# AMReX-Fluids/IAMR

Measured on AMD Instinct MI355X. Metric: cells-advanced/sec, higher is better.
Workload: dtype f64; 1 GPU; TaylorGreen 3D single level, one 256^3 box per GPU in a 1x1x1 arrangement (256x256x256 cells), periodic, nu=1e-4 cfl=0.7 Godunov_PLM be_cn_theta=0.5, full NavierStokes::advance per step

## Files before the change

iamr_amd/csrc/k_abec.hip:

```cpp
#include "kernels.h"
#include "launch.h"
#include <map>
#include <array>
#include <cstring>
#include <vector>
#include <algorithm>

namespace iamrx {

struct CfC1 { double c1[3][3]; double c2[3][3], c3[3][3]; int maxorder; int maintain; };

__device__ __forceinline__ void cf_maintain(const FabD& phi, const FabD& cfm, const BoxD& b, const CfC1& t, int i, int j, int k, double pnew)
{
    const int idx[3] = {i, j, k};
    for (int d = 0; d < 3; ++d) {
        const int NX = min(b.len(d) + 1, t.maxorder);
        if (NX < 2) continue;
        const int target = NX == 2 ? 1 : 2;
        for (int side = 0; side < 2; ++side) {
            const int s = side == 0 ? 1 : -1, f = side == 0 ? b.lo[d] : b.hi[d];
            if ((idx[d] - f) * s + 1 != target) continue;
            int g[3] = {i, j, k};
            g[d] = f - s;
            if (cfm(g[0], g[1], g[2]) != 1.0) continue;
// ... 496 lines not shown
}

__device__ __forceinline__ double rb_take(double v) { double r; asm volatile("v_mov_b64 %0, %1" : "=v"(r) : "v"(v)); return r; }

struct RbBC { int per[3]; double c1lo[3], c2lo[3], c1hi[3], c2hi[3]; int dlo[3], dhi[3]; double c3lo[3] = {0.0, 0.0, 0.0}, c3hi[3] = {0.0, 0.0, 0.0}; };
#ifndef IAMRX_RBW_EXP
#define IAMRX_RBW_EXP 0
#endif

template <bool SG, bool WALLS>
__device__ __forceinline__ double rb_update(double dhx, double dhy, double dhz, double omega,
    double p0, double pxm, double pxp, double pym, double pyp, double pzm, double pzp, double rr, double aa,
    double bxm, double bxp, double bym, double byp, double bzm, double bzp,
    double cxl, double cxh, double cyl, double cyh, double czl, double czh)
{
    const double gamma = aa + dhx * (bxm + bxp) + dhy * (bym + byp) + dhz * (bzm + bzp);
    double g_m_d = gamma;
    if (WALLS && !(IAMRX_RBW_EXP & 2)) g_m_d = gamma - (dhx * (bxm * cxl + bxp * cxh) + dhy * (bym * cyl + byp * cyh) + dhz * (bzm * czl + bzp * czh));
    const double rho = dhx * (bxm * pxm + bxp * pxp) + dhy * (bym * pym + byp * pyp) + dhz * (bzm * pzm + bzp * pzp);
    const double res = rr - (gamma * p0 - rho);
    return p0 + omega / g_m_d * res;
}

template <int BMODE, int NW, bool HASA, bool WALLS = false, bool NBR = false, bool XO = false, bool W3 = false, bool ACC = false>
__global__ void __launch_bounds__(64 * NW) k_abec_gsrb_rb(BoxD b, FabD pin, FabD pout, FabD rhs, FabD A, FabD S, double alpha,
    double dhx, double dhy, double dhz, double omega, int sig_comp, double sig_scale, BUni bu, int wpr, int tz, int nty, int zero, int comp, int xcd_chunk,
    RbBC bc = RbBC(), const BoxD* __restrict__ boxes = nullptr, const FabD* __restrict__ pint = nullptr, const FabD* __restrict__ poutt = nullptr,
    const FabD* __restrict__ rhst = nullptr, const FabD* __restrict__ At = nullptr, const FabD* __restrict__ St = nullptr, int sel = 0)
{
#if defined(__HIP_DEVICE_COMPILE__)
    constexpr bool SG = BMODE == 1;
    if (NBR) {
        const int fab = (int)blockIdx.y;
        b = boxes[fab]; pin = pint[fab]; pout = poutt[fab]; rhs = rhst[fab];
        if (HASA) A = At[fab];
        if (SG) S = St[fab];
    }
    __shared__ double RED[3][NW][64];
    __shared__ double YM[SG ? 3 : 1][SG ? NW : 1][64];
    __shared__ double YP[SG ? 3 : 1][SG ? NW : 1][64];
    __shared__ double XF[SG ? 3 : 1][SG ? NW : 1][2];
    __shared__ double BPH[2][NW][64];
    __shared__ double BSG[SG ? 2 : 1][SG ? NW : 1][64];
    const int tid = (int)threadIdx.x, lane = tid & 63, w = tid >> 6;
    const int rw = NW / wpr, r = w / wpr, xw = w - r * wpr;
    const int tile = xcd_chunk > 0 ? ((int)blockIdx.x & 7) * xcd_chunk + ((int)blockIdx.x >> 3) : (int)blockIdx.x;
    const int ty = tile % nty, tzc = tile / nty;
    const int ny = b.len(1), nz = b.len(2);
    const int k0 = b.lo[2] + tzc * tz;
    if (k0 > b.hi[2]) return;
    const int kend = min(k0 + tz - 1, b.hi[2]);
    if (NBR && sel != 0) {
        const bool bnd = XO || ty == 0 || b.lo[1] + (ty + 1) * (rw - 2) + 1 > b.hi[1] || tzc == 0 || kend + 2 > b.hi[2];
        if ((sel == 1) == bnd) return;
// ... 53 lines not shown
        if (y_g) {
            const unsigned dr = 8u * (unsigned)parq;
            if (!zero) y.p = ld1(plane(pin, qq, comp), oPy + dr);
            if (SG) y.s = ld1(plane(S, qq, sig_comp), oSy + dr);
        }
        return y;
    };
    const bool xs_on = !(IAMRX_RBW_EXP & 1) && SG && (((wlx || olx) && !hasL) || ((whx || ohx) && !hasR));
    const unsigned oSx = xs_on ? rowoff(S, ((wlx || olx) && !hasL) ? b.lo[0] - 1 : b.hi[0] + 1, j) : 0u;
    double xs_m = 0.0, xs_c = 0.0, xsN = 0.0;
    auto xsload = [&](int qq) { return xs_on ? ld1(plane(S, qq, sig_comp), oSx) : 0.0; };
    const bool xp_on = NBR && XO && ((olx && !hasL) || (ohx && !hasR));
    const unsigned oPx = xp_on ? rowoff(pin, (olx && !hasL) ? b.lo[0] - 1 : b.hi[0] + 1, j) : 0u;
    double xp_m = 0.0, xp_c = 0.0, xpN = 0.0;
    auto xpload = [&](int qq) { return xp_on ? ld1(plane(pin, qq, comp), oPx) : 0.0; };
    const bool y2_on = W3 && (atyl || atyh);
    const unsigned oP2 = y2_on ? rowoff(pin, iL, atyl ? j + 2 : j - 2) : 0u;
    D2 Y2m = Z2, Y2c = Z2, Y2N = Z2;
    auto y2load = [&](int qq) { return (y2_on && !zero) ? ldp(pin, oP2, qq, comp) : Z2; };
    auto pload = [&](int kk) { return (!zero || (NBR && (row_out || kk < b.lo[2] || kk > b.hi[2]))) ? ldp(pin, oP, kk, comp) : Z2; };
    double bn_prev = 0.0;
    D2 CN = Z2;
    auto cload = [&](int k) { return ldpair(pout.gp() + (long)pout.n[0] * pout.n[1] * (k - pout.lo[2]) + pout.cs * comp, oO); };
    auto put = [&](int k, int park, double bn, double rn) {
        v2u o;
        if (park) { o.x = bn; o.y = rn; } else { o.x = rn; o.y = bn; }
        if (ACC) { o.x = CN.l + o.x; o.y = CN.r + o.y; }
        typedef __attribute__((address_space(1))) char gwbyte;
        *(__attribute__((address_space(1))) v2u*)((gwbyte*)(pout.gp() + (long)pout.n[0] * pout.n[1] * (k - pout.lo[2]) + pout.cs * comp) + (size_t)oO) = o;
    };
    int q = k0 - 1;
    Pc = pload(q - 1); Pp = pload(q); PN = pload(q + 1);
    if (SG) { Sc = ldp(S, oS, q - 1, sig_comp); Sp = ldp(S, oS, q, sig_comp); SN = ldp(S, oS, q + 1, sig_comp); }
    Rc = ldv(rhs, oR, q - 1, comp); RN = ldv(rhs, oR, q, comp);
    if (has_a) { Ac = ldv(A, oA, q - 1, 0); AN = ldv(A, oA, q, 0); }
    YN yn, YNN = yload(q, parity(q));
    if (WALLS || (NBR && XO)) { xs_c = xsload(q - 1); xsN = xsload(q); }
    if (NBR && XO) { xp_c = xpload(q - 1); xpN = xpload(q); }
    if (W3) { Y2c = y2load(q - 1); Y2N = y2load(q); }
    {
        const int par = parity(q);
        BPH[0][w][lane] = par ? Pp.l : Pp.r;
        if (SG) BSG[0][w][lane] = par ? Sp.l : Sp.r;
        __syncthreads();
    }
    auto iter = [&](auto PARC, const int q) {
        constexpr int par = decltype(PARC)::value;
        Pm = Pc; Pc = Pp; if (!zero || NBR) { Pp.l = rb_take(PN.l); Pp.r = rb_take(PN.r); }
        if (SG) { Sm = Sc; Sc = Sp; Sp.l = rb_take(SN.l); Sp.r = rb_take(SN.r); }
        Rm = Rc; Rc.l = rb_take(RN.l); Rc.r = rb_take(RN.r);
        if (has_a) { Am = Ac; Ac.l = rb_take(AN.l); Ac.r = rb_take(AN.r); }
        yn = YNN;
        if (y_g) { if (!zero) yn.p = rb_take(YNN.p); if (SG) yn.s = rb_take(YNN.s); }
        if ((WALLS || (NBR && XO)) && SG) { xs_m = xs_c; xs_c = xs_on ? rb_take(xsN) : 0.0; }
        if (NBR && XO) { xp_m = xp_c; xp_c = xp_on ? rb_take(xpN) : 0.0; }
        if (W3) { Y2m = Y2c; if (y2_on && !zero) { Y2c.l = rb_take(Y2N.l); Y2c.r = rb_take(Y2N.r); } }
        if (owner && q - 2 >= k0) put(q - 2, par, bn_prev, RNm);
        if (q <= kend) {
            if (NBR) PN = pload(q + 2); else if (!zero) PN = ldp(pin, oP, q + 2, comp);
            if (SG) SN = ldp(S, oS, q + 2, sig_comp);
            RN = ldv(rhs, oR, q + 1, comp);
            if (has_a) AN = ldv(A, oA, q + 1, 0);
            YNN = yload(q + 1, 1 - par);
            if ((WALLS || (NBR && XO)) && SG) xsN = xsload(q + 1);
            if (NBR && XO) xpN = xpload(q + 1);
            if (W3 && y2_on && !zero) Y2N = y2load(q + 1);
        }
        if (ACC && owner && q - 1 >= k0 && q - 1 <= kend) CN = cload(q - 1);
        const int bq = (q - k0 + 1) & 1;
        const int slot = (q - k0 + 3) % 3, slotk = (q - k0 + 2) % 3;
        double bnear_c = bu.v[0], bfar_c = bu.v[0], bzp_c = bu.v[2];
        {
            double nb = par == 0 ? rb_lane_lo(Pc.r) : rb_lane_hi(Pc.l), nbs = 0.0;
            if (SG) nbs = par == 0 ? rb_lane_lo(Sc.r) : rb_lane_hi(Sc.l);
            const double p0 = par ? Pc.r : Pc.l;
            const double x2 = W3 ? (par == 0 ? rb_lane_hi(Pc.l) : rb_lane_lo(Pc.r)) : 0.0;
            double cxl = 0.0, cxh = 0.0, czl = 0.0, czh = 0.0;
            if (par == 0 ? !hasL : !hasR) {
                if (WALLS && !(IAMRX_RBW_EXP & 8) && (par == 0 ? wlx : whx)) {
                    nb = ghost3(p0, par == 0 ? Pc.r : Pc.l, x2, par == 0 ? bc.c1lo[0] : bc.c1hi[0], par == 0 ? bc.c2lo[0] : bc.c2hi[0], par == 0 ? bc.c3lo[0] : bc.c3hi[0]);
                    if (SG && !(IAMRX_RBW_EXP & 64)) nbs = xs_c;
                    if (!(IAMRX_RBW_EXP & 32)) { if (par == 0) cxl = bc.c1lo[0]; else cxh = bc.c1hi[0]; }
                } else if (NBR && XO && (par == 0 ? olx : ohx)) {
                    nb = zero ? 0.0 : xp_c;
                    if (SG) nbs = xs_c;
                } else {
// ... 304 lines not shown
{
    BUni bn;
    for (int d = 0; d < 3; ++d) bn.v[d] = c.bu[d] * ((c.tensor_eta && n == d) ? 4.0 / 3.0 : 1.0);
    return bn;
}
static RbBC comp_rbbc(const Geometry& g, const DomainBC* bcs, int nbc, int n, const CfTab* cf, const BoxD& b)
{
    RbBC r;
    for (int d = 0; d < 3; ++d) { r.per[d] = 1; r.c1lo[d] = r.c2lo[d] = r.c1hi[d] = r.c2hi[d] = 0.0; r.dlo[d] = g.domain.lo[d]; r.dhi[d] = g.domain.hi[d]; }
    if (cf) {
        for (int d = 0; d < 3; ++d) {
            const int NX = std::min(b.len(d) + 1, cf->maxorder);
            const double* w = cf->c[d][NX - 2];
            r.per[d] = 0;
            r.c1lo[d] = r.c1hi[d] = w[1];
            r.c2lo[d] = r.c2hi[d] = NX > 2 ? w[2] : 0.0;
            r.c3lo[d] = r.c3hi[d] = NX > 3 ? w[3] : 0.0;
            r.dlo[d] = b.lo[d]; r.dhi[d] = b.hi[d];
        }
    } else if (!(g.periodic[0] && g.periodic[1] && g.periodic[2])) rb_make_bc(g, bcs[n < nbc ? n : 0], r);
    return r;
}

template <int NW>
static void abec_gsrb_rb_nw(const Geometry& g, const AbecCoef& c, const MultiFab& pin, MultiFab& pout, const MultiFab& rhs, double omega, bool zero,
                            const DomainBC* bcs, int nbc, const CfTab* cf, bool acc)
{
    const bool walls = cf != nullptr || !(g.periodic[0] && g.periodic[1] && g.periodic[2]);
    auto& ctx = Context::get();
    const Layout& l = *pin.layout;
    const BoxD b = l.boxes[l.local[0]];
    const int wpr = b.len(0) / 128, rw = NW / wpr;
    const int nty = (b.len(1) + (rw - 2) - 1) / (rw - 2);
    int nch = std::max(1, (int)(tune("GSRB_RB_SLOTS", 256) / nty));
    int tz = std::max(8, (b.len(2) + nch - 1) / nch);
    nch = (b.len(2) + tz - 1) / tz;
    const int ntile = nty * nch, xcd_chunk = tune("GSRB_RB_XCD", 1) != 0 ? (ntile + 7) / 8 : 0, nwg = xcd_chunk > 0 ? 8 * xcd_chunk : ntile;
    const double dhx = c.beta / (g.dx[0] * g.dx[0]), dhy = c.beta / (g.dx[1] * g.dx[1]), dhz = c.beta / (g.dx[2] * g.dx[2]);
    const bool has_a = c.a && c.alpha != 0.0;
    const FabD P = pin.h_tab[0], O = pout.h_tab[0], R = rhs.h_tab[0], Af = has_a ? c.a->h_tab[0] : P, Sf = c.sig ? c.sig->h_tab[0] : P;
    const bool rec = !acc && pin.ncomp == 1 && kernel_probe_begin(PROBE_ABEC_GSRB, (long)l.max_len[0] * l.max_len[1] * l.max_len[2]);
    for (int n = 0; n < pin.ncomp; ++n) {
        const BUni bn = comp_buni(c, n);
        const RbBC rbc = comp_rbbc(g, bcs, nbc, n, cf, b);
#define IAMRX_RBL(M, HA, WL, T3, AC) hipLaunchKernelGGL((k_abec_gsrb_rb<M, NW, HA, WL, false, false, T3, AC>), dim3((unsigned)nwg), dim3(64 * NW), 0, ctx.stream, b, P, O, R, Af, Sf, \
                           c.alpha, dhx, dhy, dhz, omega, M == 1 ? c.sig_comp : 0, M == 1 ? c.sig_scale : 1.0, bn, wpr, tz, nty, zero ? 1 : 0, n, xcd_chunk, rbc)
#define IAMRX_RBA(M, HA, WL, T3) do { if (acc) IAMRX_RBL(M, HA, WL, T3, true); else IAMRX_RBL(M, HA, WL, T3, false); } while (0)
#define IAMRX_RB(M, HA) do { if (cf) IAMRX_RBA(M, HA, true, true); else if (walls) IAMRX_RBA(M, HA, true, false); else IAMRX_RBA(M, HA, false, false); } while (0)
        if (c.sig) IAMRX_RB(1, false); else if (has_a) IAMRX_RB(2, true); else IAMRX_RB(2, false);
#undef IAMRX_RB
#undef IAMRX_RBA
#undef IAMRX_RBL
    }
    if (rec) kernel_probe_end(PROBE_ABEC_GSRB);
}
void abec_gsrb_rb(const Geometry& g, const AbecCoef& c, const AbecSmoothPlan& p, const MultiFab& pin, MultiFab& pout, const MultiFab& rhs, double omega,
                  bool zero, const DomainBC* bcs, int nbc, const CfTab* cf, bool acc)
{
    IAMRX_ASSERT(p.path == (cf ? AbecSmoothPlan::RB_CF : AbecSmoothPlan::RB_BOX) && p.made_for(pin, rhs) && pin.d_tab != pout.d_tab && pout.ngrow >= 1 && rhs.ncomp == pin.ncomp);
    if (pin.nlocal() == 0) return;
    if (p.nw == 12) abec_gsrb_rb_nw<12>(g, c, pin, pout, rhs, omega, zero, bcs, nbc, cf, acc);
    else abec_gsrb_rb_nw<16>(g, c, pin, pout, rhs, omega, zero, bcs, nbc, cf, acc);
}

template <int NW>
static void abec_gsrb_rb_nbr_nw(const Geometry& g, const AbecCoef& c, MultiFab& pin, MultiFab& pout, const MultiFab& rhs, double omega, bool zero,
                                const DomainBC* bcs, int nbc, int sel, hipStream_t on, bool acc)
{
    const bool walls = !(g.periodic[0] && g.periodic[1] && g.periodic[2]);
    auto& ctx = Context::get();
    hipStream_t strm = on ? on : ctx.stream;
    const Layout& l = *pin.layout;
    const int nbox = l.nlocal();
    const int wpr = l.max_len[0] / 128, rw = NW / wpr;
    const int nty = (l.max_len[1] + (rw - 2) - 1) / (rw - 2);
    const int slots = (int)tune("GSRB_RB_SLOTS", 256), nz = l.max_len[2];
    int best_nch = 1;
    double best_eff = -1.0;
    for (int nch = 1; nch <= std::max(1, nz / 8); ++nch) {
        const int tzc = (nz + nch - 1) / nch;
        if ((nz + tzc - 1) / tzc != nch) continue;
        const long nwg = (long)nbox * nty * nch;
        const long rounds = (nwg + slots - 1) / slots;
        const double eff = (double)nwg / (double)(rounds * slots) * (double)tzc / (double)(tzc + 2);
        if (eff > best_eff + 1.e-9) { best_eff = eff; best_nch = nch; }
// ... 1541 lines not shown
```

iamr_amd/csrc/kernels.h:

```cpp
#pragma once
#include "core.h"
#include "mf.h"

namespace iamrx {

void launch_fill(double* p, size_t n, double v, hipStream_t s);
void launch_copy_plan(const CopyDesc* d, int nd, long maxpts, const FabD* src, const FabD* dst, int scomp, int dcomp, int nc, hipStream_t s, bool add = false);
void launch_pack(const CopyDesc* d, int nd, long maxpts, const FabD* src, double* buf, long pts_total, int scomp, int nc, hipStream_t s);
void launch_unpack(const CopyDesc* d, int nd, long maxpts, const FabD* dst, const double* buf, long pts_total, int dcomp, int nc, hipStream_t s, bool add = false);
void launch_copy_plan_w(const CopyDesc* d, const int2* w, int nw, const FabD* src, const FabD* dst, int scomp, int dcomp, int nc, hipStream_t s, bool add);
void launch_pack_w(const CopyDesc* d, const int2* w, int nw, const FabD* src, double* buf, long pts_total, int scomp, int nc, hipStream_t s);
void launch_unpack_w(const CopyDesc* d, const int2* w, int nw, const FabD* dst, const double* buf, long pts_total, int dcomp, int nc, hipStream_t s, bool add);
double reduce_norm0(const MultiFab& mf, int comp, int nc, int ng, bool global = false);
void reduce_norm0_comps(const MultiFab& mf, int comp, int nc, int ng, double* out, bool global = false);
void reduce_minmax(const MultiFab& mf, int comp, int ng, double& mn, double& mx, bool global = true);
double reduce_sum_unique(const MultiFab& mf, int comp, const Geometry& g, bool global = false);
void reduce_sum_integrated(const MultiFab& S, int rho_comp, int trac_comp, const MultiFab* cov, double out[3]);
constexpr int SUM_COMPS_MAX = 8;
void reduce_sum_comps(const MultiFab& mf, int n, const int* comps, const MultiFab* cov, double* out);
void reduce_dots(int nout, const MultiFab* const* x, const MultiFab* const* y, int comp, int nc, const Geometry& g, double* out, bool local = false);
void reduce_dots_dev(int nout, const MultiFab* const* x, const MultiFab* const* y, int comp, int nc, const Geometry& g, double* d_out, bool local = false);
enum { PROBE_NODAL_GS4 = 0, PROBE_ABEC_GSRB = 1, PROBE_GOD_Z = 2, PROBE_PRED_Z = 3, PROBE_COUNT = 4 };
void kernel_probe_start(int which, long min_points, int stride);
void kernel_probe_stop(int which, double* total_ms, long* launches);
// ... 176 lines not shown
};
AbecSmoothPlan abec_smooth_plan(const Geometry& g, const AbecLevel& lv);
AbecColourForm abec_colour_form(const Geometry& g, const AbecLevel& lv, bool wrap = false, bool walls_inkernel = false);
void abec_gsrb(const Geometry& g, const AbecCoef& c, const AbecColourForm& f, MultiFab& phi, const MultiFab& rhs, int redblack, double omega,
               const DomainBC* bcs, int nbc, bool shell_only = false, bool phi_is_zero = false, const MultiFab* cfm = nullptr, const CfTab* cftab = nullptr);
bool abec_tail_ok(const Geometry& gF, const Layout& lF, const Geometry& gC, const Layout& lC, const AbecCoef& cF, const DomainBC* bcs, int nbc, int ncomp);
void abec_tail_solve(const Geometry& gF, const AbecCoef& cF, MultiFab& corF, const MultiFab& resF, const Geometry& gC, const AbecCoef& cC,
                     const DomainBC& bc, bool singular, double eps_rel, int maxiter, int nub, int nuf, int nu1, int nu2, double omega, int* d_iters);
constexpr int LEG_R = 16;
struct AbecLegPlan {
    bool on = false;
    int mode = 0;
    int tile_down[3] = {0, 0, 0}, tile_up[3] = {0, 0, 0};
    int halo_down = 0, halo_up = 0;
};
AbecLegPlan abec_leg_plan(const Geometry& g, const AbecLevel& lv, int level, int nu1, int nu2, bool slab_transition, bool agg_transition);
void abec_leg_down(const Geometry& g, const AbecCoef& c, const AbecLegPlan& p, MultiFab& buf, const MultiFab& rhs, MultiFab& crse_rhs, int nu1, double omega);
void abec_leg_up(const Geometry& g, const AbecCoef& c, const AbecLegPlan& p, MultiFab& cor, const MultiFab& buf, const MultiFab& rhs, const MultiFab& crse_cor, int nu2,
                 double omega);
bool abec_residual_reads_no_ghosts(const Geometry& g, const AbecCoef& c, const MultiFab& out, const MultiFab& phi, const MultiFab& rhs, bool restrict_form);
bool abec_resid_restrict_ok(const AbecCoef& c, const MultiFab& phi, const MultiFab& rhs);
void abec_resid_restrict(const Geometry& g, const AbecCoef& c, MultiFab& crse, const MultiFab& phi, const MultiFab& rhs);
void abec_gsrb_rb(const Geometry& g, const AbecCoef& c, const AbecSmoothPlan& p, const MultiFab& pin, MultiFab& pout, const MultiFab& rhs, double omega,
                  bool zero, const DomainBC* bcs = nullptr, int nbc = 0, const CfTab* cf = nullptr, bool acc = false);
void abec_gsrb_rb_nbr(const Geometry& g, const AbecCoef& c, const AbecSmoothPlan& p, MultiFab& pin, MultiFab& pout, const MultiFab& rhs, double omega,
                      bool zero, const DomainBC* bcs, int nbc, int sel = 0, hipStream_t on = nullptr, bool acc = false);
bool abec_gsrb_rb_ok(const Geometry& g, const AbecCoef& c, const MultiFab& phi, int nbc, const DomainBC* bcs = nullptr);
bool abec_gsrb_rb_cf_ok(const Geometry& g, const AbecCoef& c, const MultiFab& phi);
bool abec_gsrb_rb_nbr_ok(const Geometry& g, const AbecCoef& c, const MultiFab& phi, const MultiFab& rhs, int nbc, const DomainBC* bcs);
bool abec_gsrb_rb_nbr_level_ok(const Geometry& g, const Layout& l, int ncomp, bool sig_form, bool has_a, int nbc, const DomainBC* bcs);
void abec_gsrb_fused(const Geometry& g, const AbecCoef& c, const MultiFab& phi_in, MultiFab& phi_out, const MultiFab& rhs, double omega,
                     const DomainBC* bcs, int nbc);
void abec_residual(const Geometry& g, const AbecCoef& c, MultiFab& out, const MultiFab& phi, const MultiFab* rhs, double* norm_out = nullptr);
bool abec_bottom_device_ok(const Geometry& g, const Layout& l, const DomainBC* bcs, int nbc, int ncomp, bool cf = false);
void abec_bottom_solve(const Geometry& g, const AbecCoef& c, MultiFab& cor, const MultiFab& res, const DomainBC& bc, bool singular,
                       double eps_rel, int maxiter, int nub, int nuf, double omega, int* d_iters, const CfTab* cftab = nullptr);
void abec_apply_domain_bc(const Geometry& g, MultiFab& phi, const DomainBC& bc, bool inhomog, const MultiFab* bcval, int comp0 = 0, int ncomp = -1);
void abec_apply_domain_bc_percomp(const Geometry& g, MultiFab& phi, const DomainBC* bcs, int ncomp, bool inhomog, const MultiFab* bcval);
void cc_restrict(MultiFab& crse, const MultiFab& fine);
void cc_prolong_add(MultiFab& fine, const MultiFab& crse);
void face_avgdown(MultiFab& crse, const MultiFab& fine, int dir);
void abec_flux(const Geometry& g, const AbecCoef& c, const MultiFab& phi, MultiFab* const flux[3], MultiFab* const add_to[3]);
void mac_rhs(const Geometry& g, MultiFab& rhs, const MultiFab* const umac[3], const MultiFab* S, double* sum = nullptr);
void mac_bcoef(MultiFab* const b[3], const MultiFab& rho, int rho_comp, double scale);
void mac_bcoef_avgdown(MultiFab& crse, const MultiFab& rho, int rho_comp, double scale, int dir);
void abec_flux_sig(const Geometry& g, double beta, const MultiFab& rho, int rho_comp, double scale, const MultiFab& phi, MultiFab* const flux[3],
                   MultiFab* const add_to[3]);
// ... 81 lines not shown
```

iamr_amd/csrc/mlmg.h:

```cpp
#pragma once
#include <functional>
#include "mf.h"
#include "kernels.h"
#include <vector>
#include <memory>

namespace iamrx {

inline bool mg_stalled_at_floor(const std::vector<double>& hist, double r0, double target, bool fast)
{
    const size_t n = hist.size();
    if (n == 0 || !(hist[n - 1] <= 10.0 * target)) return false;
    if (n >= 4 && hist[n - 1] > 0.9 * hist[n - 4]) return true;
    if (!fast || n < 2) return false;
    const double last = hist[n - 1] / hist[n - 2];
    double best = 1.0, prev = r0;
    for (size_t i = 0; i + 1 < n; ++i) { if (prev > 0.0) best = std::min(best, hist[i] / prev); prev = hist[i]; }
    return last > 0.5 && best < 0.2;
}


struct MGOpts {
    int nu1 = 2, nu2 = 2, nuf = 8, nub = 0;
    int max_iters = 200;
// ... 80 lines not shown
    CellMG(const Geometry& g, LayoutP layout, int ncomp, const DomainBC& bc, const MGOpts& o);
    void setScalars(double alpha, double beta) { m_alpha = alpha; m_beta = beta; }
    void setACoeffs(const MultiFab* a) { m_a0 = a; }
    void setBCoeffs(const MultiFab* const b[3]) { for (int d = 0; d < 3; ++d) m_b0[d] = b[d]; }
    void setBCoeffsFromCell(const MultiFab* sig, int comp, double scale) { m_sig = sig; m_sig_comp = comp; m_sig_scale = scale; }
    void setTensor(bool t) { m_tensor = t; }
    void setTensorEta(bool t) { m_tensor_eta = t; }
    void setDomainBCs(const DomainBC* bcs, int n) { m_bcn.assign(bcs, bcs + n); }
    void setCoarseFineBC(const MultiFab* crse, const Geometry& cgeom, int ratio) { m_cf = true; m_crse = crse; m_cgeom = cgeom; m_ratio = ratio; }
    void prepare();
    void prepareBoundary();
    void fillBoundaryData(MultiFab& phi);
    MGStats solve(MultiFab& phi, const MultiFab& rhs, double rtol, double atol) { return solve_on(phi, rhs, nullptr, rtol, atol, nullptr); }
    MGStats solve_giving_rhs(MultiFab& phi, MultiFab& rhs, double rtol, double atol, const double* rhs_sum = nullptr) { return solve_on(phi, rhs, &rhs, rtol, atol, rhs_sum); }
    bool singular() const { return m_singular; }
    void apply(MultiFab& out, MultiFab& phi);
    void fluxes(MultiFab& phi, MultiFab* const flux[3], MultiFab* const add_to[3]);
    int nlevels() const { return (int)m_lev.size(); }
    AbecCoef coef(int l) const;
    AbecCoef smoother_coef(int l) const;
    const Geometry& geom(int l) const { return m_lev[l].g; }
    void applyBC(int l, MultiFab& phi, bool inhomog, const MultiFab* bcval, bool corners = true);
    void smooth(int l, bool skip_fill, bool cf_ghosts_current = false, bool sol_is_zero = false);
    void smooth_n(int l, int nsweeps, bool skip_first_fill, bool sol_is_zero = false, MultiFab* acc = nullptr);
    void vcycle(MGStats& st);
    MultiFab& res(int l) { return m_lev[l].res; }
    MultiFab& cor(int l) { return m_lev[l].cor; }

private:
    struct Level : MGLevel {
        MultiFab a, b[3];
        MultiFab cor, res, rescor;
        MultiFab buf;
        AbecSmoothPlan plan;
        AbecLegPlan legs;
        MultiFab cfm;
        CfTab cftab;
    };
    MGStats solve_on(MultiFab& phi, const MultiFab& rhs_in, MultiFab* rhs_mine, double rtol, double atol, const double* rhs_sum);
    int bicgstab(int l, MultiFab& sol, const MultiFab& rhs, double eps_rel, double eps_abs, int& niters);
    void bottom_solve(MGStats& st);
    template <class Sweep> void pingpong(MultiFab& sol, MultiFab& buf, int nsweeps, bool sol_is_zero, MultiFab* acc, Sweep sweep);
    bool tail_fused() const;
    void cf_bcval(MultiFab& bcval);
    void prepare_cf(int l);
    void subtract_mean(int l, MultiFab& mf);
    Geometry m_g;
// ... 82 lines not shown
```

iamr_amd/csrc/mlmg.hip:

```cpp
#include "mlmg.h"
#include "krylov.h"
#include "launch.h"
#include <chrono>
#include <cmath>

namespace iamrx {

void parallel_copy(MultiFab& dst, const MultiFab& src, int scomp, int dcomp, int nc, int src_ng, int dst_ng, const Geometry* periodic_geom, bool add);

CycleTimer& cycle_timer() { static CycleTimer t; return t; }

long mg_agglomeration_cells() { return (long)tune("MG_AGGLOMERATE_CELLS", 2097152.0); }

bool mg_agglomerate_level(const Layout& c)
{
    if (c.replicated || c.total_cells() > mg_agglomeration_cells()) return false;
    if (Context::get().comm->nranks > 1) return true;
    return c.boxes.size() > 1 && tune("MG_AGG_SINGLE_RANK", 1) != 0;
}

bool mg_slab_level(const Geometry& g, const Layout& l, int min_width, bool slab_problem)
{
    if (!slab_problem && tune("MG_SLAB", 0) == 0) return false;
    if (!g.periodic[1] || g.domain.lo[1] != 0 || g.domain.hi[1] != 1) return false;
// ... 289 lines not shown
            } else applyBC(l, sol, false, nullptr, false);
        }
        abec_gsrb(L.g, smoother_coef(l), f, sol, L.res, rb, m_dd_sweeps > 0 ? dd_omega() : m_o.omega, m_bcn.data(), (int)m_bcn.size(), false, sol_is_zero && rb == 0,
                  m_cf ? &L.cfm : nullptr, m_cf ? &L.cftab : nullptr);
        skip_fill = false;
    }
}

template <class Sweep>
void CellMG::pingpong(MultiFab& sol, MultiFab& buf, int nsweeps, bool sol_is_zero, MultiFab* acc, Sweep sweep)
{
    MultiFab* a = &sol;
    MultiFab* b = &buf;
    if (sol_is_zero && (nsweeps & 1)) std::swap(a, b);
    for (int i = 0; i < nsweeps; ++i) {
        const bool last = acc && i == nsweeps - 1;
        sweep(*a, last ? *acc : *b, sol_is_zero && i == 0, last);
        if (last) { m_acc_done = true; return; }
        std::swap(a, b);
    }
    if (a != &sol) MultiFab::Copy(sol, *a, 0, 0, m_ncomp, 0);
}

void CellMG::smooth_n(int l, int nsweeps, bool skip_first_fill, bool sol_is_zero, MultiFab* acc)
{
    Level& L = m_lev[l];
    MultiFab& sol = L.cor;
    const MultiFab& rhs = L.res;
    const AbecSmoothPlan& plan = L.plan;
    IAMRX_ASSERT(plan.made_for(sol, rhs));
    if (l != 0) acc = nullptr;
    if (nsweeps <= 0) { if (sol_is_zero) sol.setVal(0.0); return; }
    const AbecCoef c = smoother_coef(l);
    const DomainBC* bcs = m_bcn.data();
    const int nbc = (int)m_bcn.size();
    const double om = m_dd_sweeps > 0 ? dd_omega() : m_o.omega;
    if (plan.path != AbecSmoothPlan::COLOUR && (!L.buf.defined() || L.buf.ngrow != sol.ngrow)) L.buf.define(L.layout, cell_type(), m_ncomp, sol.ngrow);
    switch (plan.path) {
    case AbecSmoothPlan::COLOUR:
        for (int i = 0; i < nsweeps; ++i) smooth(l, skip_first_fill && i == 0, i > 0, sol_is_zero && i == 0);
        return;
    case AbecSmoothPlan::RB_BOX:
    case AbecSmoothPlan::RB_CF:
        pingpong(sol, L.buf, nsweeps, sol_is_zero, acc, [&](MultiFab& in, MultiFab& out, bool zero, bool last) {
            abec_gsrb_rb(L.g, c, plan, in, out, rhs, om, zero, bcs, nbc, plan.path == AbecSmoothPlan::RB_CF ? &L.cftab : nullptr, last);
        });
        return;
    case AbecSmoothPlan::RB_NBR: {
        if (!L.res_filled) {
            const int one[3] = {1, 1, 1};
            L.res.FillBoundary(L.g, 0, m_ncomp, one);
            L.res_filled = true;
        }
        auto& ctx = Context::get();
        const int ov_mode = (int)tune("HALO_OVERLAP", 1);
        const CopyPlan& fplan = fill_boundary_plan(*L.layout, cell_type(), sol.ngrow, L.g);
        const bool overlap = ov_mode != 0 && (ov_mode == 2 || !fplan.peers.empty()) && plan.nbr_splits;
        pingpong(sol, L.buf, nsweeps, sol_is_zero, acc, [&](MultiFab& in, MultiFab& out, bool z, bool last) {
            if (z || !overlap) {
                if (!z) in.FillBoundary(L.g);
                abec_gsrb_rb_nbr(L.g, c, plan, in, out, rhs, om, z, bcs, nbc, 0, nullptr, last);
            } else {
                ctx.fork_side();
                abec_gsrb_rb_nbr(L.g, c, plan, in, out, rhs, om, false, bcs, nbc, 1, ctx.stream, last);
                in.FillBoundary(L.g, 0, m_ncomp, nullptr, -1, ctx.side);
                abec_gsrb_rb_nbr(L.g, c, plan, in, out, rhs, om, false, bcs, nbc, 2, ctx.side, last);
                ctx.join_side();
            }
// ... 231 lines not shown
        Level& C = m_lev[l + 1];
        mg_restrict_to(C, C.res, C.tmp_d, C.vres, [&](MultiFab& target) {
            if (abec_resid_restrict_ok(cl, L.cor, L.res)) abec_resid_restrict(L.g, cl, target, L.cor, L.res);
            else {
                level_residual(L.g, cl, L.rescor, L.cor, &L.res);
                cc_restrict(target, L.rescor);
            }
        });
    }
    if (tail) {
        Level& F = m_lev[nl - 2];
        Level& C = m_lev[nl - 1];
        const int maxiter = krylov_maxiter(m_o.bottom_maxiter, C.layout->total_cells() * m_ncomp);
        abec_tail_solve(F.g, smoother_coef(nl - 2), F.cor, F.res, C.g, smoother_coef(nl - 1), m_bcn[0], m_singular, m_o.bottom_reltol, maxiter, m_o.nub, m_o.nuf,
                        m_o.nu1, m_o.nu2, m_o.omega, mg_bottom_iters_dev());
    } else
    bottom_solve(st);
    for (int l = nsm - 1; l >= 0; --l) {
        Level& L = m_lev[l];
        if (L.legs.on) {
            abec_leg_up(L.g, smoother_coef(l), L.legs, L.cor, L.buf, L.res, m_lev[l + 1].cor, m_o.nu2, m_o.omega);
            continue;
        }
        cc_prolong_add(L.cor, mg_correction_of(m_lev[l + 1], m_lev[l + 1].cor, 0));
        smooth_n(l, m_o.nu2, false, false, l == 0 ? m_acc : nullptr);
    }
}

void CellMG::fillBoundaryData(MultiFab& phi)
{
    const Geometry& g0 = m_lev[0].g;
    if (m_cf || !(g0.periodic[0] && g0.periodic[1] && g0.periodic[2])) {
        MultiFab bcval(m_lev[0].layout, cell_type(), m_ncomp, 1);
        MultiFab::Copy(bcval, phi, 0, 0, m_ncomp, 1);
        cf_bcval(bcval);
        applyBC(0, phi, true, &bcval);
    } else applyBC(0, phi, true, nullptr);
}

void CellMG::apply(MultiFab& out, MultiFab& phi)
{
    fillBoundaryData(phi);
    level_residual(m_lev[0].g, coef(0), out, phi, nullptr);
}

void CellMG::fluxes(MultiFab& phi, MultiFab* const flux[3], MultiFab* const add_to[3])
{
    if (m_sig && m_ncomp == 1 && (!m_b0[0] || tune("MAC_GLUE", 1) != 0)) {
// ... 108 lines not shown
```

iamr_amd/csrc/navierstokes.hip:

```cpp
#include "operators.h"
#include "particles.h"
#include "launch.h"
#include <cmath>
#include <chrono>

namespace iamrx {

namespace {
struct SectionTimer {
    NavierStokes& ns; int idx; bool on;
    std::chrono::steady_clock::time_point t0;
    SectionTimer(NavierStokes& n, int i) : ns(n), idx(i), on(n.profile_sections)
    {
        if (on) { Context::get().sync(); t0 = std::chrono::steady_clock::now(); }
    }
    ~SectionTimer()
    {
        if (on) { Context::get().sync(); ns.t_sections[idx] += std::chrono::duration<double, std::milli>(std::chrono::steady_clock::now() - t0).count(); }
    }
};
}

static LayoutP level_work_layout(const Geometry& geom, const LayoutP& lay)
{
// ... 425 lines not shown
    MultiFab r;
    crse_state_at(r, t, Density, 1);
    const FabD *ot = out.d_tab, *rt = r.d_tab;
    for_each(*crse->layout, cell_type(), 0, Context::get().stream, [=] __device__(int i, int j, int k, int f) { ot[f](i, j, k) /= rt[f](i, j, k); });
}

void NavierStokes::fill_gradp_bc()
{
    fill_gp(Gp[pnew], 0.5 * (pt_new[0] + pt_new[1]));
}

static void floor_small(MultiFab& mf)
{
    const FabD* t = mf.d_tab;
    const int nc = mf.ncomp;
    for_each(*mf.layout, mf.type, mf.ngrow, Context::get().stream, [=] __device__(int i, int j, int k, int f) {
        const FabD a = t[f];
        for (int n = 0; n < nc; ++n) { const double v = a(i, j, k, n); if (fabs(v) <= 1.e-20) a(i, j, k, n) = 0.0; }
    });
}

void NavierStokes::compute_visc_terms_vel(MultiFab& visc, MultiFab& Sdata)
{
    visc.setVal(1.e40);
    if (!is_diffusive_vel()) { visc.setVal(0.0); return; }
    MultiFab stmp(layout, cell_type(), 3, 1);
    fillpatch(stmp, Sdata, Xvel, 3, bc_vel);
    const MultiFab* ep[3];
    MultiFab eta_les[3];
    get_viscosity(ep, eta_les, Sdata);
    MultiFab cdata;
    TensorCF cf{&cdata, level > 0 ? &crse->g : nullptr, ratio};
    if (level > 0) crse_state_at(cdata, state_time(Sdata), Xvel, 3);
    tensor_apply(g, visc, stmp, 0.0, -1.0, nullptr, ep, bc_visc, 3, level > 0 ? &cf : nullptr);
    visc.FillBoundary(g);
    first_order_extrap(visc);
}

void NavierStokes::calc_mut_LES(MultiFab out[3], MultiFab& Sdata)
{
    MultiFab vel(layout, cell_type(), 3, 1);
    fillpatch(vel, Sdata, Xvel, 3, bc_vel);
    MultiFab cdata;
    TensorCF cf{&cdata, level > 0 ? &crse->g : nullptr, ratio};
    if (level > 0) crse_state_at(cdata, state_time(Sdata), Xvel, 3);
    DomainBC bl[3];
    for (int n = 0; n < 3; ++n) { bl[n] = bc_visc[n]; bl[n].maxorder = 3; }
    MultiFab* mp[3];
// ... 49 lines not shown
}

const MultiFab& NavierStokes::old_visc_or_zero(MultiFab& scratch)
{
    if (p.be_cn_theta != 1.0) return visc_terms_vel_old(scratch);
    scratch.define(layout, cell_type(), 3, 1);
    scratch.setVal(0.0);
    return scratch;
}

void scale_by(MultiFab& y, const MultiFab& x, int xcomp, int ng, bool divide)
{
    const FabD *yt = y.d_tab, *xt = x.d_tab;
    for_each(*y.layout, cell_type(), ng, Context::get().stream, [=] __device__(int i, int j, int k, int f) {
        const double r = xt[f](i, j, k, xcomp);
        if (divide) yt[f](i, j, k, 0) /= r; else yt[f](i, j, k, 0) *= r;
    });
}

void NavierStokes::get_visc_terms_scalar(MultiFab& visc, MultiFab& Sdata, int comp)
{
    const int sn = comp - Density;
    const bool over_rho = scal_rho_flag[sn] == 2;
    visc.setVal(1.e40);
    if (!is_diffusive_scal(comp)) { visc.setVal(0.0); return; }
    MultiFab stmp(layout, cell_type(), 1, 1);
    fillpatch(stmp, Sdata, comp, 1, &bc_scal[sn]);
    if (over_rho) scale_by(stmp, rho_ptime, 0, 1, true);
    MGOpts mo;
    mo.max_coarsening_level = 0;
    mo.maxorder = 2;
    CellMG mg(g, layout, 1, bc_scal_lin[sn], mo);
    mg.setScalars(0.0, -1.0);
    const MultiFab* bp[3] = {&diff_b[sn][0], &diff_b[sn][1], &diff_b[sn][2]};
    mg.setBCoeffs(bp);
    MultiFab cdata;
    if (level > 0) {
        crse_scalar_at(cdata, state_time(Sdata), comp, over_rho);
        mg.setCoarseFineBC(&cdata, crse->g, ratio);
    }
    mg.prepare();
    MultiFab tmp(layout, cell_type(), 1, 0);
    mg.apply(tmp, stmp);
    MultiFab::Copy(visc, tmp, 0, 0, 1, 0);
    visc.FillBoundary(g);
    first_order_extrap(visc);
}

// ... 964 lines not shown
```

Measured before the change: 518.8 million cells/s.

## Fuse MG piecewise-constant prolongation into the first red-black GS sweep

On the V-cycle up leg, the coarse correction is now added inside the first red-black smoother sweep when the level is periodic, single-box, 2:1 aligned and uses NW=16. The kernel reads the coarse cell per fine row and adds it to the loaded phi, which removes the separate cc_prolong_add pass over the fine correction. This adds a template variant and a gated path, and it is controlled by a tuning knob. It also moves the early return in the visc-term functions ahead of a redundant setVal.

```diff
diff --git a/iamr_amd/csrc/k_abec.hip b/iamr_amd/csrc/k_abec.hip
--- a/iamr_amd/csrc/k_abec.hip
+++ b/iamr_amd/csrc/k_abec.hip
@@ -542,14 +542,17 @@
     return p0 + omega / g_m_d * res;
 }
 
-template <int BMODE, int NW, bool HASA, bool WALLS = false, bool NBR = false, bool XO = false, bool W3 = false, bool ACC = false>
+template <int BMODE, int NW, bool HASA, bool WALLS = false, bool NBR = false, bool XO = false, bool W3 = false, bool ACC = false, bool PRO = false>
 __global__ void __launch_bounds__(64 * NW) k_abec_gsrb_rb(BoxD b, FabD pin, FabD pout, FabD rhs, FabD A, FabD S, double alpha,
     double dhx, double dhy, double dhz, double omega, int sig_comp, double sig_scale, BUni bu, int wpr, int tz, int nty, int zero, int comp, int xcd_chunk,
     RbBC bc = RbBC(), const BoxD* __restrict__ boxes = nullptr, const FabD* __restrict__ pint = nullptr, const FabD* __restrict__ poutt = nullptr,
-    const FabD* __restrict__ rhst = nullptr, const FabD* __restrict__ At = nullptr, const FabD* __restrict__ St = nullptr, int sel = 0)
+    const FabD* __restrict__ rhst = nullptr, const FabD* __restrict__ At = nullptr, const FabD* __restrict__ St = nullptr, int sel = 0,
+    FabD crs = FabD())
 {
 #if defined(__HIP_DEVICE_COMPILE__)
     constexpr bool SG = BMODE == 1;
+    static_assert(!PRO || !(WALLS || NBR || XO || W3), "PRO: index-wrap levels only");
+    static_assert(!(PRO && ACC && BMODE == 1), "PRO with ACC: the density form would spill");
     if (NBR) {
         const int fab = (int)blockIdx.y;
         b = boxes[fab]; pin = pint[fab]; pout = poutt[fab]; rhs = rhst[fab];
@@ -649,6 +652,9 @@
     double bn_prev = 0.0;
     D2 CN = Z2;
     auto cload = [&](int k) { return ldpair(pout.gp() + (long)pout.n[0] * pout.n[1] * (k - pout.lo[2]) + pout.cs * comp, oO); };
+    const unsigned oC = PRO ? rowoff(crs, iL >> 1, j >> 1) : 0u;
+    auto crsload = [&](int kk) { return ld1(crs.gp() + (long)crs.n[0] * crs.n[1] * ((wk(kk) >> 1) - crs.lo[2]) + crs.cs * comp, oC); };
+    double CRN = 0.0, CRp = 0.0;
     auto put = [&](int k, int park, double bn, double rn) {
         v2u o;
         if (park) { o.x = bn; o.y = rn; } else { o.x = rn; o.y = bn; }
@@ -665,6 +671,12 @@
     if (WALLS || (NBR && XO)) { xs_c = xsload(q - 1); xsN = xsload(q); }
     if (NBR && XO) { xp_c = xpload(q - 1); xpN = xpload(q); }
     if (W3) { Y2c = y2load(q - 1); Y2N = y2load(q); }
+    if (PRO) {
+        const double cm = crsload(q - 1);
+        CRp = crsload(q);
+        Pc.l = Pc.l + cm; Pc.r = Pc.r + cm; Pp.l = Pp.l + CRp; Pp.r = Pp.r + CRp;
+        CRN = crsload(q + 1);
+    }
     {
         const int par = parity(q);
         BPH[0][w][lane] = par ? Pp.l : Pp.r;
@@ -674,11 +686,13 @@
     auto iter = [&](auto PARC, const int q) {
         constexpr int par = decltype(PARC)::value;
         Pm = Pc; Pc = Pp; if (!zero || NBR) { Pp.l = rb_take(PN.l); Pp.r = rb_take(PN.r); }
+        const double cry = CRp;
+        if (PRO) { CRp = rb_take(CRN); Pp.l = Pp.l + CRp; Pp.r = Pp.r + CRp; }
         if (SG) { Sm = Sc; Sc = Sp; Sp.l = rb_take(SN.l); Sp.r = rb_take(SN.r); }
         Rm = Rc; Rc.l = rb_take(RN.l); Rc.r = rb_take(RN.r);
         if (has_a) { Am = Ac; Ac.l = rb_take(AN.l); Ac.r = rb_take(AN.r); }
         yn = YNN;
-        if (y_g) { if (!zero) yn.p = rb_take(YNN.p); if (SG) yn.s = rb_take(YNN.s); }
+        if (y_g) { if (!zero) yn.p = rb_take(YNN.p); if (SG) yn.s = rb_take(YNN.s); if (PRO) yn.p = yn.p + cry; }
         if ((WALLS || (NBR && XO)) && SG) { xs_m = xs_c; xs_c = xs_on ? rb_take(xsN) : 0.0; }
         if (NBR && XO) { xp_m = xp_c; xp_c = xp_on ? rb_take(xpN) : 0.0; }
         if (W3) { Y2m = Y2c; if (y2_on && !zero) { Y2c.l = rb_take(Y2N.l); Y2c.r = rb_take(Y2N.r); } }
@@ -689,6 +703,7 @@
             RN = ldv(rhs, oR, q + 1, comp);
             if (has_a) AN = ldv(A, oA, q + 1, 0);
             YNN = yload(q + 1, 1 - par);
+            if (PRO) CRN = crsload(q + 2);
             if ((WALLS || (NBR && XO)) && SG) xsN = xsload(q + 1);
             if (NBR && XO) xpN = xpload(q + 1);
             if (W3 && y2_on && !zero) Y2N = y2load(q + 1);
@@ -1039,9 +1054,19 @@
     return r;
 }
 
+bool abec_gsrb_rb_pro_ok(const Geometry& g, const AbecCoef& c, const AbecSmoothPlan& p, const MultiFab& fine, const MultiFab& crse, bool acc)
+{
+    if (acc && c.sig) return false;
+    if (p.path != AbecSmoothPlan::RB_BOX || p.nw != 16 || !(g.periodic[0] && g.periodic[1] && g.periodic[2])) return false;
+    if (fine.nlocal() != 1 || crse.nlocal() != 1 || crse.ncomp != fine.ncomp) return false;
+    const BoxD f = fine.layout->boxes[fine.layout->local[0]], cb = crse.layout->boxes[crse.layout->local[0]];
+    for (int d = 0; d < 3; ++d) if ((f.lo[d] & 1) || (f.len(d) & 1) || cb.lo[d] != (f.lo[d] >> 1) || cb.hi[d] != (f.hi[d] >> 1)) return false;
+    return true;
+}
+
 template <int NW>
 static void abec_gsrb_rb_nw(const Geometry& g, const AbecCoef& c, const MultiFab& pin, MultiFab& pout, const MultiFab& rhs, double omega, bool zero,
-                            const DomainBC* bcs, int nbc, const CfTab* cf, bool acc)
+                            const DomainBC* bcs, int nbc, const CfTab* cf, bool acc, const MultiFab* pro)
 {
     const bool walls = cf != nullptr || !(g.periodic[0] && g.periodic[1] && g.periodic[2]);
     auto& ctx = Context::get();
@@ -1056,15 +1081,22 @@
     const double dhx = c.beta / (g.dx[0] * g.dx[0]), dhy = c.beta / (g.dx[1] * g.dx[1]), dhz = c.beta / (g.dx[2] * g.dx[2]);
     const bool has_a = c.a && c.alpha != 0.0;
     const FabD P = pin.h_tab[0], O = pout.h_tab[0], R = rhs.h_tab[0], Af = has_a ? c.a->h_tab[0] : P, Sf = c.sig ? c.sig->h_tab[0] : P;
-    const bool rec = !acc && pin.ncomp == 1 && kernel_probe_begin(PROBE_ABEC_GSRB, (long)l.max_len[0] * l.max_len[1] * l.max_len[2]);
+    const FabD C = pro ? pro->h_tab[0] : P;
+    const bool rec = !acc && !pro && pin.ncomp == 1 && kernel_probe_begin(PROBE_ABEC_GSRB, (long)l.max_len[0] * l.max_len[1] * l.max_len[2]);
     for (int n = 0; n < pin.ncomp; ++n) {
         const BUni bn = comp_buni(c, n);
         const RbBC rbc = comp_rbbc(g, bcs, nbc, n, cf, b);
-#define IAMRX_RBL(M, HA, WL, T3, AC) hipLaunchKernelGGL((k_abec_gsrb_rb<M, NW, HA, WL, false, false, T3, AC>), dim3((unsigned)nwg), dim3(64 * NW), 0, ctx.stream, b, P, O, R, Af, Sf, \
-                           c.alpha, dhx, dhy, dhz, omega, M == 1 ? c.sig_comp : 0, M == 1 ? c.sig_scale : 1.0, bn, wpr, tz, nty, zero ? 1 : 0, n, xcd_chunk, rbc)
-#define IAMRX_RBA(M, HA, WL, T3) do { if (acc) IAMRX_RBL(M, HA, WL, T3, true); else IAMRX_RBL(M, HA, WL, T3, false); } while (0)
+#define IAMRX_RBL(M, HA, WL, T3, AC, PR) hipLaunchKernelGGL((k_abec_gsrb_rb<M, NW, HA, WL, false, false, T3, AC, PR>), dim3((unsigned)nwg), dim3(64 * NW), 0, ctx.stream, b, P, O, R, Af, Sf, \
+                           c.alpha, dhx, dhy, dhz, omega, M == 1 ? c.sig_comp : 0, M == 1 ? c.sig_scale : 1.0, bn, wpr, tz, nty, zero ? 1 : 0, n, xcd_chunk, rbc, \
+                           nullptr, nullptr, nullptr, nullptr, nullptr, nullptr, 0, C)
+#define IAMRX_RBA(M, HA, WL, T3) do { if (acc) IAMRX_RBL(M, HA, WL, T3, true, false); else IAMRX_RBL(M, HA, WL, T3, false, false); } while (0)
 #define IAMRX_RB(M, HA) do { if (cf) IAMRX_RBA(M, HA, true, true); else if (walls) IAMRX_RBA(M, HA, true, false); else IAMRX_RBA(M, HA, false, false); } while (0)
+#define IAMRX_RBP(M, HA) do { if (acc) IAMRX_RBL(M, HA, false, false, true, true); else IAMRX_RBL(M, HA, false, false, false, true); } while (0)
+        if (pro) {
+            if constexpr (NW == 16) { if (c.sig) IAMRX_RBL(1, false, false, false, false, true); else if (has_a) IAMRX_RBP(2, true); else IAMRX_RBP(2, false); }
+        } else
         if (c.sig) IAMRX_RB(1, false); else if (has_a) IAMRX_RB(2, true); else IAMRX_RB(2, false);
+#undef IAMRX_RBP
 #undef IAMRX_RB
 #undef IAMRX_RBA
 #undef IAMRX_RBL
@@ -1072,12 +1104,13 @@
     if (rec) kernel_probe_end(PROBE_ABEC_GSRB);
 }
 void abec_gsrb_rb(const Geometry& g, const AbecCoef& c, const AbecSmoothPlan& p, const MultiFab& pin, MultiFab& pout, const MultiFab& rhs, double omega,
-                  bool zero, const DomainBC* bcs, int nbc, const CfTab* cf, bool acc)
+                  bool zero, const DomainBC* bcs, int nbc, const CfTab* cf, bool acc, const MultiFab* pro)
 {
     IAMRX_ASSERT(p.path == (cf ? AbecSmoothPlan::RB_CF : AbecSmoothPlan::RB_BOX) && p.made_for(pin, rhs) && pin.d_tab != pout.d_tab && pout.ngrow >= 1 && rhs.ncomp == pin.ncomp);
     if (pin.nlocal() == 0) return;
-    if (p.nw == 12) abec_gsrb_rb_nw<12>(g, c, pin, pout, rhs, omega, zero, bcs, nbc, cf, acc);
-    else abec_gsrb_rb_nw<16>(g, c, pin, pout, rhs, omega, zero, bcs, nbc, cf, acc);
+    IAMRX_ASSERT(!pro || (!zero && !cf && abec_gsrb_rb_pro_ok(g, c, p, pin, *pro, acc)));
+    if (p.nw == 12) abec_gsrb_rb_nw<12>(g, c, pin, pout, rhs, omega, zero, bcs, nbc, cf, acc, pro);
+    else abec_gsrb_rb_nw<16>(g, c, pin, pout, rhs, omega, zero, bcs, nbc, cf, acc, pro);
 }
 
 template <int NW>
diff --git a/iamr_amd/csrc/kernels.h b/iamr_amd/csrc/kernels.h
--- a/iamr_amd/csrc/kernels.h
+++ b/iamr_amd/csrc/kernels.h
@@ -222,7 +222,8 @@
 bool abec_resid_restrict_ok(const AbecCoef& c, const MultiFab& phi, const MultiFab& rhs);
 void abec_resid_restrict(const Geometry& g, const AbecCoef& c, MultiFab& crse, const MultiFab& phi, const MultiFab& rhs);
 void abec_gsrb_rb(const Geometry& g, const AbecCoef& c, const AbecSmoothPlan& p, const MultiFab& pin, MultiFab& pout, const MultiFab& rhs, double omega,
-                  bool zero, const DomainBC* bcs = nullptr, int nbc = 0, const CfTab* cf = nullptr, bool acc = false);
+                  bool zero, const DomainBC* bcs = nullptr, int nbc = 0, const CfTab* cf = nullptr, bool acc = false, const MultiFab* pro = nullptr);
+bool abec_gsrb_rb_pro_ok(const Geometry& g, const AbecCoef& c, const AbecSmoothPlan& p, const MultiFab& fine, const MultiFab& crse, bool acc);
 void abec_gsrb_rb_nbr(const Geometry& g, const AbecCoef& c, const AbecSmoothPlan& p, MultiFab& pin, MultiFab& pout, const MultiFab& rhs, double omega,
                       bool zero, const DomainBC* bcs, int nbc, int sel = 0, hipStream_t on = nullptr, bool acc = false);
 bool abec_gsrb_rb_ok(const Geometry& g, const AbecCoef& c, const MultiFab& phi, int nbc, const DomainBC* bcs = nullptr);
diff --git a/iamr_amd/csrc/mlmg.h b/iamr_amd/csrc/mlmg.h
--- a/iamr_amd/csrc/mlmg.h
+++ b/iamr_amd/csrc/mlmg.h
@@ -126,7 +126,7 @@
     const Geometry& geom(int l) const { return m_lev[l].g; }
     void applyBC(int l, MultiFab& phi, bool inhomog, const MultiFab* bcval, bool corners = true);
     void smooth(int l, bool skip_fill, bool cf_ghosts_current = false, bool sol_is_zero = false);
-    void smooth_n(int l, int nsweeps, bool skip_first_fill, bool sol_is_zero = false, MultiFab* acc = nullptr);
+    void smooth_n(int l, int nsweeps, bool skip_first_fill, bool sol_is_zero = false, MultiFab* acc = nullptr, const MultiFab* pro = nullptr);
     void vcycle(MGStats& st);
     MultiFab& res(int l) { return m_lev[l].res; }
     MultiFab& cor(int l) { return m_lev[l].cor; }
diff --git a/iamr_amd/csrc/mlmg.hip b/iamr_amd/csrc/mlmg.hip
--- a/iamr_amd/csrc/mlmg.hip
+++ b/iamr_amd/csrc/mlmg.hip
@@ -335,7 +335,7 @@
     if (a != &sol) MultiFab::Copy(sol, *a, 0, 0, m_ncomp, 0);
 }
 
-void CellMG::smooth_n(int l, int nsweeps, bool skip_first_fill, bool sol_is_zero, MultiFab* acc)
+void CellMG::smooth_n(int l, int nsweeps, bool skip_first_fill, bool sol_is_zero, MultiFab* acc, const MultiFab* pro)
 {
     Level& L = m_lev[l];
     MultiFab& sol = L.cor;
@@ -343,6 +343,7 @@
     const AbecSmoothPlan& plan = L.plan;
     IAMRX_ASSERT(plan.made_for(sol, rhs));
     if (l != 0) acc = nullptr;
+    IAMRX_ASSERT(!pro || (plan.path == AbecSmoothPlan::RB_BOX && nsweeps >= 1 && !sol_is_zero));
     if (nsweeps <= 0) { if (sol_is_zero) sol.setVal(0.0); return; }
     const AbecCoef c = smoother_coef(l);
     const DomainBC* bcs = m_bcn.data();
@@ -356,7 +357,9 @@
     case AbecSmoothPlan::RB_BOX:
     case AbecSmoothPlan::RB_CF:
         pingpong(sol, L.buf, nsweeps, sol_is_zero, acc, [&](MultiFab& in, MultiFab& out, bool zero, bool last) {
-            abec_gsrb_rb(L.g, c, plan, in, out, rhs, om, zero, bcs, nbc, plan.path == AbecSmoothPlan::RB_CF ? &L.cftab : nullptr, last);
+            abec_gsrb_rb(L.g, c, plan, in, out, rhs, om, zero, bcs, nbc, plan.path == AbecSmoothPlan::RB_CF ? &L.cftab : nullptr, last, pro);
+            if (pro) tuning_count("MG_PRO_SWEEP_COUNT");
+            pro = nullptr;
         });
         return;
     case AbecSmoothPlan::RB_NBR: {
@@ -634,8 +637,11 @@
             abec_leg_up(L.g, smoother_coef(l), L.legs, L.cor, L.buf, L.res, m_lev[l + 1].cor, m_o.nu2, m_o.omega);
             continue;
         }
-        cc_prolong_add(L.cor, mg_correction_of(m_lev[l + 1], m_lev[l + 1].cor, 0));
-        smooth_n(l, m_o.nu2, false, false, l == 0 ? m_acc : nullptr);
+        const MultiFab& crse = mg_correction_of(m_lev[l + 1], m_lev[l + 1].cor, 0);
+        MultiFab* const acc = l == 0 ? m_acc : nullptr;
+        const bool pro = m_o.nu2 >= 1 && tune("MG_PRO_SWEEP", 1) != 0 && abec_gsrb_rb_pro_ok(L.g, smoother_coef(l), L.plan, L.cor, crse, acc && m_o.nu2 == 1);
+        if (!pro) cc_prolong_add(L.cor, crse);
+        smooth_n(l, m_o.nu2, false, false, acc, pro ? &crse : nullptr);
     }
 }
 
diff --git a/iamr_amd/csrc/navierstokes.hip b/iamr_amd/csrc/navierstokes.hip
--- a/iamr_amd/csrc/navierstokes.hip
+++ b/iamr_amd/csrc/navierstokes.hip
@@ -471,8 +471,8 @@
 
 void NavierStokes::compute_visc_terms_vel(MultiFab& visc, MultiFab& Sdata)
 {
+    if (!is_diffusive_vel()) { visc.setVal(0.0); return; }
     visc.setVal(1.e40);
-    if (!is_diffusive_vel()) { visc.setVal(0.0); return; }
     MultiFab stmp(layout, cell_type(), 3, 1);
     fillpatch(stmp, Sdata, Xvel, 3, bc_vel);
     const MultiFab* ep[3];
@@ -568,8 +568,8 @@
 {
     const int sn = comp - Density;
     const bool over_rho = scal_rho_flag[sn] == 2;
+    if (!is_diffusive_scal(comp)) { visc.setVal(0.0); return; }
     visc.setVal(1.e40);
-    if (!is_diffusive_scal(comp)) { visc.setVal(0.0); return; }
     MultiFab stmp(layout, cell_type(), 1, 1);
     fillpatch(stmp, Sdata, comp, 1, &bc_scal[sn]);
     if (over_rho) scale_by(stmp, rho_ptime, 0, 1, true);
```

Result: faster. 525.6 million cells/s (median of 6 runs) (+1.3%).
